# lh3/minigraph

Measured on NVIDIA H100. Metric: mapped Gbp/s (-cx lr), higher is better.
Workload: dtype int64/u8 (fp32 chain penalties, bit-exact)

## Files before the change

### minigraph_b200/csrc/mgb_common.cuh

```cuda
#pragma once
#include <stdint.h>
#include <stddef.h>
#include <string.h>

#if defined(__CUDACC__)
#define MG_HD __host__ __device__
#define MG_D __device__
#else
#define MG_HD
#define MG_D
#endif

#if defined(__CUDA_ARCH__)
#define MGB_ON_DEVICE 1
#else
#define MGB_ON_DEVICE 0
#endif

#if defined(__CUDACC__)
#define MG_NOINLINE __noinline__
#define MGB_NO_UNROLL _Pragma("unroll 1")
#else
#define MG_NOINLINE __attribute__((noinline))
#define MGB_NO_UNROLL
// ... 308 lines not shown
}
MG_HD inline int nth_set_bit(uint32_t mask, int k)
{
#if MGB_ON_DEVICE
	const unsigned r = __fns(mask, 0, k);
	return r > 31? 32 : (int)r;
#else
	for (int b = 0; b < 32; ++b) if ((mask >> b & 1) && --k == 0) return b;
	return 32;
#endif
}
MG_HD inline int replay_skips(uint32_t imp, uint32_t mk, int max_skip, int32_t *n_skip)
{
	int32_t ns = *n_skip;
	for (;;) {
		const int nxt = imp? ctz32_nz(imp) : 32;
		const uint32_t seg = nxt >= 32? mk : mk & ((1u << nxt) - 1u);
		const int c = mask_count(seg);
		if (ns + c > max_skip) { *n_skip = max_skip + 1; return nth_set_bit(seg, max_skip - ns + 1); }
		ns += c;
		if (nxt >= 32) break;
		if (ns > 0) --ns;
		imp &= imp - 1, mk &= ~((2u << nxt) - 1u);
	}
	*n_skip = ns;
	return -1;
}
MG_HD inline int ctz32(uint32_t x)
{
#if MGB_ON_DEVICE
	return __ffs((int)x) - 1;
#else
	return __builtin_ctz(x);
#endif
}

MG_HD inline int nt4(uint8_t c)
{
	const uint32_t idx = c & 0x1fu;
	const uint64_t code = (1ULL << 2 * 3) | (2ULL << 2 * 7) | (3ULL << 2 * 20) | (3ULL << 2 * 21);
	const uint32_t letters = (1u << 1) | (1u << 3) | (1u << 7) | (1u << 20) | (1u << 21);
	if ((c & 0xc0u) == 0x40u && (letters >> idx & 1u)) return (int)(code >> 2 * idx & 3u);
	return c < 4? (int)c : 4;
}

template<typename T, typename KeyFn>
MG_HD inline void rs_insertsort(T *beg, T *end, KeyFn key)
{
	for (T *i = beg + 1; i < end; ++i) {
		if (key(*i) < key(*(i - 1))) {
			T *j, tmp = *i;
			for (j = i; j > beg && key(tmp) < key(*(j - 1)); --j) *j = *(j - 1);
			*j = tmp;
		}
	}
}

struct RsRange { int32_t beg, end, s; };

template<typename T, typename KeyFn>
MG_HD inline int radix_sort_exact(Arena &A, T *a, int64_t n, int sizeof_key, KeyFn key)
{
	const int MIN_SIZE = 64;
	if (n <= MIN_SIZE) { rs_insertsort(a, a + n, key); return 0; }
	uint64_t mark = A.top;
	RsRange *stack;
// ... 205 lines not shown
```

### minigraph_b200/csrc/mgb_galign.cuh

```cuda
#pragma once
#include "mgb_pipeline.cuh"
#include "mgb_gchain.cuh"
#include "mgb_wfa_tiers.cuh"
#if defined(MGB_HOSTSIM)
#include <stdio.h>
#include <stdlib.h>
#endif

namespace mgb {

MG_HD inline int cigar_append1(Arena &A, AVec<uint64_t> &c, int32_t op, int32_t len)
{
	if (c.n > 0 && (int32_t)(c.a[c.n - 1] & 0xf) == op) c.a[c.n - 1] += (uint64_t)(int64_t)len << 4;
	else {
		uint64_t x = (uint64_t)(int64_t)len << 4 | (uint64_t)op;
		MGB_TRY(avec_push(A, c, x));
	}
	return 0;
}

MG_HD inline int cigar_append(Arena &A, AVec<uint64_t> &c, int32_t n_cigar, const uint32_t *cigar)
{
	if (n_cigar == 0) return 0;
	MGB_TRY(cigar_append1(A, c, (int32_t)(cigar[0] & 0xf), (int32_t)(cigar[0] >> 4)));
// ... 63 lines not shown
	const char *tseq;
	if (l == l0) tseq = g_vseq(g, lc[l0].v) + J->t_beg;
	else {
		char *seq;
		MGB_ALLOC(A, seq, char, tl + 1);
		int32_t n = g_vlen(g, lc[l0].v) - J->t_beg, at = 0;
		const char *s = g_vseq(g, lc[l0].v) + J->t_beg;
		for (int32_t x = lane; x < n; x += MGB_W) seq[at + x] = s[x];
		at += n;
		for (int32_t k = l0 + 1; k < l; ++k) {
			s = g_vseq(g, lc[k].v), n = g_vlen(g, lc[k].v);
			for (int32_t x = lane; x < n; x += MGB_W) seq[at + x] = s[x];
			at += n;
		}
		s = g_vseq(g, lc[l].v), n = J->t_last + 1;
		for (int32_t x = lane; x < n; x += MGB_W) seq[at + x] = s[x];
		at += n;
		if (at != tl) return MGB_E_INTERNAL;
		warp_sync();
		tseq = seq;
	}
	WfResult rst;
	unsigned long long pt0 = prof_clock();
	int rc;
	if (tier == 1) rc = wfa_smem<WfTier1::W_, WfTier1::MAXLEN_, WfTier1::TBCAP_>(A, smem, tl, tseq, ql, qs, &rst, lane);
	else if (tier == 2) rc = wfa_smem<WfTier2::W_, WfTier2::MAXLEN_, WfTier2::TBCAP_>(A, smem, tl, tseq, ql, qs, &rst, lane);
	else rc = wfa_exact(A, tl, tseq, ql, qs, 100000000LL, &rst, lane);
	if (rc < 0) return rc;
	if (lane == 0) {
		unsigned long long dt = prof_clock() - pt0;
		int slot = tier == 1? PROF_WFA_FAST_CYC : tier == 2? PROF_WFA_MID_CYC : PROF_WFA_SLOW_CYC;
		prof_add(c, slot, dt), prof_add(c, slot + 1, 1);
		prof_max(c, PROF_WFA_MAX_CYC, dt << 16 | (unsigned long long)(mlen < 65535? mlen : 65535));
		if (rc == 0) prof_add(c, PROF_WFA_CELLS, (unsigned long long)rst.n_iter);
		if (rc == 0 && explore && c.tier_hist) {
			unsigned int *h = &c.tier_hist[(mlen >> 4 < 31? mlen >> 4 : 31) * 4 + tier];
#if MGB_ON_DEVICE
			atomicAdd(h, 1u);
#else
			++*h;
#endif
		}
	}
	if (rc == 1) {
		if (lane == 0) {
			unsigned int at;
#if MGB_ON_DEVICE
			at = atomicAdd(&c.jobq_n[tier - 1], 1u);
#else
			at = c.jobq_n[tier - 1]++;
#endif
			c.jobq[tier - 1][at] = (int32_t)job_idx;
		}
		return 0;
	}
	if (rst.s < 0) return MGB_E_INTERNAL;
	int64_t coff = 0;
	if (lane == 0) {
#if MGB_ON_DEVICE
		unsigned long long *ck = wfa_cig_chunk(smem, tier);
		const unsigned long long need = ((unsigned long long)rst.n_cigar * 4 + 15) & ~15ULL;
		if (ck == 0) coff = pool_alloc(c.pool_cig, (uint64_t)rst.n_cigar * 4);
		else if (ck[0] + need > ck[1]) {
			const unsigned long long get = need > CIG_CHUNK_BYTES? need : CIG_CHUNK_BYTES;
			const int64_t off = pool_alloc(c.pool_cig, get);
			if (off < 0) ck[0] = ck[1] = 0;
			else ck[0] = (unsigned long long)off, ck[1] = (unsigned long long)off + get;
// ... 617 lines not shown
```

### minigraph_b200/csrc/mgb_pipeline.cuh

```cuda
#pragma once
#include "mgb_model.cuh"
#include "mgb_seed.cuh"
#include "mgb_lchain.cuh"
#include "mgb_gclabel.cuh"
#include "mgb_tma.cuh"

namespace mgb {

struct PipeCtx {
	GraphDev g;
	IndexDev ix;
	MapOptDev opt;
	BatchDev b;
	ReadMeta *meta;
	Pool *pool_anchor;     u128 *anchor;
	Pool *pool_minipos;    int32_t *minipos;
	Pool *pool_lchain;     LChain *lchain;
	Pool *pool_out;        char *out;
	Pool *pool_plan;       uint64_t *plan;
	Pool *pool_jobs;       struct WfaJob *jobs;
	Pool *pool_cig;        uint32_t *cig;
	int32_t *jobq[2];      unsigned int *jobq_n;
	Pool *pool_gstate;     char *gstate;
	Pool *pool_gjobs;      struct GwfaJob *gjobs;
	Pool *pool_walk;       int32_t *walk;
	int32_t *rescue_list;  unsigned int *rescue_n;
	LabTab lab;
	unsigned int *next_read;
	unsigned long long *prof;
	int32_t skip1_len, skip2_len;
	unsigned int *tier_hist;
};

enum { PROF_WFA_FAST_CYC = 0, PROF_WFA_FAST_N, PROF_WFA_SLOW_CYC, PROF_WFA_SLOW_N, PROF_WFA_MAX_CYC, PROF_WFA_CELLS, PROF_WFA_TB_CYC,
	   PROF_GC_DP_CYC, PROF_GC_GEN_CYC, PROF_GC_POST_CYC, PROF_GC_PLAN_CYC, PROF_FIN_CIGAR_CYC, PROF_FIN_DS_CYC, PROF_SEED_SKETCH_CYC,
	   PROF_SEED_MATCH_CYC, PROF_SEED_SORT_CYC, PROF_CHAIN_DP_CYC, PROF_CHAIN_BT_CYC, PROF_CHAIN_RMQ_CYC, PROF_CHAIN_POST_CYC, PROF_WFA_MID_CYC, PROF_WFA_MID_N, PROF_GC_GWFA_CYC, PROF_GC_SHORTK_CYC, PROF_GC_EXTRA_CYC, PROF_GWFA_MAX_CYC, PROF_GC_DP_MAX_CYC, PROF_WFA_CTA_CYC, PROF_WFA_CTA_N, PROF_LAB_CYC, PROF_LAB_N, PROF_N = 32 };

MG_HD inline unsigned long long prof_clock()
{
#if MGB_ON_DEVICE
	return (unsigned long long)clock64();
#else
	return 0;
#endif
}
#if defined(__CUDACC__)
MG_D inline unsigned long long *prof_block() { __shared__ unsigned long long s_prof[PROF_N]; return s_prof; }
MG_D inline bool prof_is_max(int slot) { return slot == PROF_WFA_MAX_CYC || slot == PROF_GWFA_MAX_CYC || slot == PROF_GC_DP_MAX_CYC; }
MG_D inline void prof_block_begin() { if (threadIdx.x < PROF_N) prof_block()[threadIdx.x] = 0; __syncthreads(); }
MG_D inline void prof_block_end(unsigned long long *prof)
{
	__syncthreads();
	if (prof && threadIdx.x < PROF_N) {
		const unsigned long long v = prof_block()[threadIdx.x];
		if (v) { if (prof_is_max((int)threadIdx.x)) atomicMax(&prof[threadIdx.x], v); else atomicAdd(&prof[threadIdx.x], v); }
	}
}
#endif
MG_HD inline void prof_add(const PipeCtx &c, int slot, unsigned long long v)
{
#if MGB_ON_DEVICE
	if (c.prof) atomicAdd(&prof_block()[slot], v);
#else
	if (c.prof) c.prof[slot] += v;
#endif
}
MG_HD inline void prof_max(const PipeCtx &c, int slot, unsigned long long v)
{
#if MGB_ON_DEVICE
	if (c.prof) atomicMax(&prof_block()[slot], v);
#else
	if (c.prof && c.prof[slot] < v) c.prof[slot] = v;
#endif
}

MG_HD inline int stage_seed(const PipeCtx &c, int rid, Arena &A, int lane, int32_t *smem = 0)
{
	ReadMeta &m = c.meta[rid];
// ... 281 lines not shown
```

### minigraph_b200/csrc/mgb_wfa.cuh

```cuda
#pragma once
#include "mgb_common.cuh"

namespace mgb {

static const int32_t WF_NEG_INF = -0x40000000;
static const int WF_X = 4, WF_O1 = 4, WF_E1 = 2, WF_O2 = 15, WF_E2 = 1;
static const int WF_MAX_PEN = 16;
static const int WF_NSLICE = WF_MAX_PEN + 1;
static const int WF_PAD = WF_MAX_PEN + 1;
static const int WF_SEQ_PAD = 16;

#define MGB_WF_MAX(a, b) ((a) >= (b)? (a) : (b))

struct WfResult {
	int32_t s;
	int32_t n_cigar;
	int64_t n_iter;
	uint32_t *cigar;
};


MG_HD inline void wf_stage_seq(char *dst, const char *src, int32_t len, uint8_t sentinel, int lane)
{
	for (int32_t i = lane; i < len; i += MGB_W) dst[i] = src[i];
	for (int32_t i = len + lane; i < len + WF_SEQ_PAD; i += MGB_W) dst[i] = (char)sentinel;
}

MG_HD inline uint32_t wf_ld32u(const char *base, int32_t pos)
{
	const uint32_t *w = (const uint32_t*)base;
	uint32_t lo = w[pos >> 2], hi = w[(pos >> 2) + 1];
	int sh = (pos & 3) << 3;
#if MGB_ON_DEVICE
	return __funnelshift_r(lo, hi, sh);
#else
	return sh? (lo >> sh) | (hi << (32 - sh)) : lo;
#endif
}

MG_HD inline int32_t wf_extend(const char *ts, const char *qs, int32_t k, int32_t d)
{
	for (;;) {
		uint32_t x = wf_ld32u(ts, k + 1) ^ wf_ld32u(qs, d + k + 1);
		if (x) {
#if MGB_ON_DEVICE
			return k + ((__ffs((int)x) - 1) >> 3);
#else
			return k + (__builtin_ctz(x) >> 3);
#endif
		}
		k += 4;
	}
}

template<typename TB>
MG_HD inline int wf_traceback(const TB &tb, int32_t n_scores, int32_t tl, const char *ts, int32_t ql, const char *qs, int32_t last_state,
							  uint32_t *cig_store, int64_t max_cigar, int32_t *n_cigar, int64_t *first)
{
	int32_t i = ql - 1, k = tl - 1, s = n_scores - 1, last = last_state;
	int64_t w = max_cigar;
	int32_t cur_op = -1, cur_len = 0;
#define MGB_CIG_PUSH(op_, len_) do { \
		if (cur_op == (op_)) cur_len += (len_); \
		else { \
			if (cur_op >= 0) { if (w <= 0) return MGB_E_INTERNAL; cig_store[--w] = (uint32_t)cur_len << 4 | (uint32_t)cur_op; } \
			cur_op = (op_), cur_len = (len_); \
		} \
	} while (0)
	while (i >= 0 && k >= 0) {
		int32_t k0 = k, x, state, ext;
		if (last == 0) {
			while (i >= 0 && k >= 0 && qs[i] == ts[k]) --i, --k;
			if (k0 - k > 0) MGB_CIG_PUSH(7, k0 - k);
			if (i < 0 || k < 0) break;
		}
		if (s < 0) return MGB_E_INTERNAL;
		x = tb.get(s, i - k);
		if (x < 0) return MGB_E_INTERNAL;
		state = last == 0? x & 7 : last;
		ext = state > 0? x >> (state + 2) & 1 : 0;
		if (state == 0) { MGB_CIG_PUSH(8, 1); --i, --k, s -= WF_X; }
		else if (state == 1) { MGB_CIG_PUSH(1, 1); --i, s -= ext? WF_E1 : WF_O1 + WF_E1; }
		else if (state == 3) { MGB_CIG_PUSH(1, 1); --i, s -= ext? WF_E2 : WF_O2 + WF_E2; }
		else if (state == 2) { MGB_CIG_PUSH(2, 1); --k, s -= ext? WF_E1 : WF_O1 + WF_E1; }
		else if (state == 4) { MGB_CIG_PUSH(2, 1); --k, s -= ext? WF_E2 : WF_O2 + WF_E2; }
		else return MGB_E_INTERNAL;
		last = state > 0 && ext? state : 0;
	}
	if (i >= 0) MGB_CIG_PUSH(1, i + 1);
	else if (k >= 0) MGB_CIG_PUSH(2, k + 1);
	if (cur_op >= 0) { if (w <= 0) return MGB_E_INTERNAL; cig_store[--w] = (uint32_t)cur_len << 4 | (uint32_t)cur_op; }
#undef MGB_CIG_PUSH
	*n_cigar = (int32_t)(max_cigar - w), *first = w;
	return 0;
}


typedef int16_t wf_cell_t;
static const int32_t WF_NEG_INF16 = -30000;

template<int W, int MAXLEN, int TBCAP, int HS = 17>
struct WfSmemLayout {
	static const int W_ = W, MAXLEN_ = MAXLEN, TBCAP_ = TBCAP, HS_ = HS;
	static const int N_CELLS = (HS + 3 + 3 + 2 + 2) * W;
	static const int N_INTS = N_CELLS / 2;
	static const int SEQ_BYTES = (MAXLEN + WF_SEQ_PAD + 3) / 4 * 4;
// ... 148 lines not shown
	x |= pHo2[d+1] >= pF2[d+1]? 0 : 0x40;
	f2 = MGB_WF_MAX(pHo2[d+1], pF2[d+1]) + 1;
	zf = f1 >= f2? 2 : 4;
	f = MGB_WF_MAX(f1, f2);
	z = e >= f? ze : zf;
	h = MGB_WF_MAX(e, f);
	z = pHx[d] + 1 >= h? 0 : z;
	E1[d] = e1, E2[d] = e2, F1[d] = f1, F2[d] = f2;
	H[d] = MGB_WF_MAX(pHx[d] + 1, h);
	return x | z;
}

struct WfChkpt { int32_t s, d; };

MG_HD inline int wfa_core(Arena &A, int32_t tl, const char *ts, int32_t ql, const char *qs, int64_t max_iter, int32_t n_seg, const WfChkpt *seg,
						  WfResult *r, uint32_t *cig_store, int64_t max_cigar, int lane, int nl)
{
	uint64_t mark = A.top;
	WfState wf;
	int32_t last_state = 0, stopped = 0, sid = 0;
	MGB_TRY(wf_state_alloc(A, wf, tl, ql));
	AVec<WfTbRow> rows;
	avec_init(rows);
	if (nl > 1) MGB_TRY(avec_reserve_w(A, rows, 1024, lane));
	else MGB_TRY(avec_reserve(A, rows, 1024));
	wf_stripe_init(wf, lane, nl);
	for (;;) {
		WfSlice *p = &wf.sl[wf.top];
		int32_t lo, hi, *H = p->H;
		int hit = 0, hit_noext = 0;
		for (int32_t d = p->lo + lane; d <= p->hi; d += nl) {
			int32_t k0 = H[d];
			if (k0 < -1 || d + k0 < -1 || k0 >= tl || d + k0 >= ql) continue;
			int32_t k = wf_extend(ts, qs, k0, d);
			if (k == tl - 1 && d + k == ql - 1) { hit = 1, hit_noext = (k == k0); if (nl == 1) break; }
			else H[d] = k;
		}
		MGB_NL_SYNC(nl);
		if (nl > 1? warp_any(hit) : hit) {
			if (nl > 1? warp_any(hit && hit_noext) : hit_noext) {
				WfTbArena t; t.row = rows.a;
				last_state = t.get((int32_t)rows.n - 1, ql - tl) & 7;
			}
			break;
		}
		if (seg && sid < n_seg && seg[sid].s == wf.s) {
			if (!(seg[sid].d >= wf.lo && seg[sid].d <= wf.hi)) { A.top = mark; return MGB_E_INTERNAL; }
			wf.lo = wf.hi = seg[sid++].d;
		}
		lo = wf.lo > -tl? wf.lo - 1 : -tl;
		hi = wf.hi < ql? wf.hi + 1 : ql;
		{
			const WfSlice &ft = wf_stripe_add(wf, lo, hi, lane, nl);
			const WfSlice &fx = wf_stripe_get(wf, WF_X);
			const WfSlice &fo1 = wf_stripe_get(wf, WF_O1 + WF_E1);
			const WfSlice &fo2 = wf_stripe_get(wf, WF_O2 + WF_E2);
			const WfSlice &fe1 = wf_stripe_get(wf, WF_E1);
			const WfSlice &fe2 = wf_stripe_get(wf, WF_E2);
			if (nl > 1) MGB_TRY(avec_reserve_w(A, rows, rows.n + 1, lane));
			else MGB_TRY(avec_reserve(A, rows, rows.n + 1));
			uint8_t *x;
			MGB_ALLOC(A, x, uint8_t, hi - lo + 1);
			if (lane == 0) rows.a[rows.n].lo = lo, rows.a[rows.n].hi = hi, rows.a[rows.n].x = x;
			++rows.n;
			uint8_t *ax = x - lo;
			for (int32_t dd = lo + lane; dd <= hi; dd += nl)
				ax[dd] = wf_cell(dd, ft.H, ft.E1, ft.F1, ft.E2, ft.F2, fx.H, fo1.H, fo2.H, fe1.E1, fe1.F1, fe2.E2, fe2.F2);
			MGB_NL_SYNC(nl);
			if (ft.H[lo] >= -1 || ft.E1[lo] >= -1 || ft.F1[lo] >= -1 || ft.E2[lo] >= -1 || ft.F2[lo] >= -1) wf.lo = lo;
			if (ft.H[hi] >= -1 || ft.E1[hi] >= -1 || ft.F1[hi] >= -1 || ft.E2[hi] >= -1 || ft.F2[hi] >= -1) wf.hi = hi;
		}
		if ((wf.s & 0xff) == 0) MGB_TRY(wf_stripe_shrink(wf, tl, ql));
		r->n_iter += hi - lo + 1;
		if (max_iter > 0 && r->n_iter > max_iter) { stopped = 1; break; }
	}
	r->s = stopped? -1 : wf.s;
	if (!stopped) {
		int rc = 0;
		int32_t n_cig = 0;
		int64_t first = 0;
		if (lane == 0) {
			WfTbArena t; t.row = rows.a;
			rc = wf_traceback(t, (int32_t)rows.n, tl, ts, ql, qs, last_state, cig_store, max_cigar, &n_cig, &first);
		}
		if (nl > 1) {
			rc = warp_bcast_i32(rc, 0), n_cig = warp_bcast_i32(n_cig, 0), first = (int64_t)warp_bcast_u64((uint64_t)first, 0);
			warp_sync();
		}
		if (rc < 0) { A.top = mark; return rc; }
		r->n_cigar = n_cig, r->cigar = cig_store + first;
	}
	A.top = mark;
	return 0;
}


struct WfSnap { int32_t n, n_intv, max_s; int32_t *x; uint64_t *intv; };

MG_HD inline int wf_snapshot(Arena &A, AVec<WfSnap> &sss, WfState &sf)
{
	WfSnap ss;
	int32_t j, k, t;
	ss.n = 0, ss.max_s = sf.s;
	for (j = 0; j < WF_NSLICE; ++j) ss.n += 5 * (sf.sl[j].hi - sf.sl[j].lo + 1);
	MGB_ALLOC(A, ss.x, int32_t, ss.n);
	ss.n_intv = WF_NSLICE;
	MGB_ALLOC(A, ss.intv, uint64_t, ss.n_intv);
	for (j = 0, t = 0; j < WF_NSLICE; ++j) {
		WfSlice *p = &sf.sl[(sf.top + 1 + j) % WF_NSLICE];
		ss.intv[j] = (uint64_t)(int64_t)p->lo << 32 | (uint64_t)(uint32_t)((p->hi - p->lo + 1) * 5);
		for (k = p->lo; k <= p->hi; ++k) {
			ss.x[t] = p->H[k],  p->H[k]  = t++;
			ss.x[t] = p->E1[k], p->E1[k] = t++;
			ss.x[t] = p->F1[k], p->F1[k] = t++;
			ss.x[t] = p->E2[k], p->E2[k] = t++;
			ss.x[t] = p->F2[k], p->F2[k] = t++;
		}
	}
	if (t != ss.n) return MGB_E_INTERNAL;
	return avec_push(A, sss, ss);
}

MG_HD inline int wfa_seg(Arena &A, int32_t step, int32_t tl, const char *ts, int32_t ql, const char *qs, WfChkpt **seg_, int32_t *n_seg_)
{
	uint64_t mark = A.top;
	WfState wf, sf;
	AVec<WfSnap> sss;
	uint8_t *xbuf;
	int32_t last = -1;
	avec_init(sss);
	*seg_ = 0, *n_seg_ = 0;
	MGB_ALLOC(A, xbuf, uint8_t, (int64_t)tl + ql + 1);
	MGB_TRY(wf_state_alloc(A, wf, tl, ql));
	MGB_TRY(wf_state_alloc(A, sf, tl, ql));
	wf_stripe_init(wf, 0, 1);
	wf_stripe_init(sf, 0, 1);
	for (;;) {
		WfSlice *p = &wf.sl[wf.top];
		int32_t d, lo, hi, *H = p->H;
		for (d = p->lo; d <= p->hi; ++d) {
			int32_t k0 = H[d];
			if (k0 < -1 || d + k0 < -1 || k0 >= tl || d + k0 >= ql) continue;
			int32_t k = wf_extend(ts, qs, k0, d);
			if (k == tl - 1 && d + k == ql - 1) { last = sf.sl[sf.top].H[d]; break; }
			H[d] = k;
		}
		if (d <= p->hi) break;
		lo = wf.lo > -tl? wf.lo - 1 : -tl;
		hi = wf.hi < ql? wf.hi + 1 : ql;
		if ((wf.s + 1) % step == 0) MGB_TRY(wf_snapshot(A, sss, sf));
		{
			uint8_t *ax = xbuf - lo;
			{
				const WfSlice &ft = wf_stripe_add(wf, lo, hi, 0, 1);
				const WfSlice &fx = wf_stripe_get(wf, WF_X), &fo1 = wf_stripe_get(wf, WF_O1 + WF_E1), &fo2 = wf_stripe_get(wf, WF_O2 + WF_E2);
				const WfSlice &fe1 = wf_stripe_get(wf, WF_E1), &fe2 = wf_stripe_get(wf, WF_E2);
				for (int32_t dd = lo; dd <= hi; ++dd)
					ax[dd] = wf_cell(dd, ft.H, ft.E1, ft.F1, ft.E2, ft.F2, fx.H, fo1.H, fo2.H, fe1.E1, fe1.F1, fe2.E2, fe2.F2);
			}
			const WfSlice &gt = wf_stripe_add(sf, lo, hi, 0, 1);
			const WfSlice &gx = wf_stripe_get(sf, WF_X), &go1 = wf_stripe_get(sf, WF_O1 + WF_E1), &go2 = wf_stripe_get(sf, WF_O2 + WF_E2);
			const WfSlice &ge1 = wf_stripe_get(sf, WF_E1), &ge2 = wf_stripe_get(sf, WF_E2);
			for (int32_t dd = lo; dd <= hi; ++dd) {
				uint8_t x = ax[dd];
				int32_t e1, f1, e2, f2, h;
				e1 = gt.E1[dd] = (x & 0x08) == 0? go1.H[dd-1] : ge1.E1[dd-1];
				f1 = gt.F1[dd] = (x & 0x10) == 0? go1.H[dd+1] : ge1.F1[dd+1];
				e2 = gt.E2[dd] = (x & 0x20) == 0? go2.H[dd-1] : ge2.E2[dd-1];
				f2 = gt.F2[dd] = (x & 0x40) == 0? go2.H[dd+1] : ge2.F2[dd+1];
				x &= 7;
				h = gx.H[dd];
				h = x == 1? e1 : h;
				h = x == 2? f1 : h;
				h = x == 3? e2 : h;
				h = x == 4? f2 : h;
				gt.H[dd] = h;
// ... 221 lines not shown
				}
				r->s += q.s;
				A.top = m2;
			}
		} else if (x0 < x1) {
			MGB_TRY(wf_cig_push1(cig_store, &nc, max_cigar, 2, x1 - x0));
			r->s += WF_O2 + (x1 - x0) * WF_E2 < WF_O1 + (x1 - x0) * WF_E1? WF_O2 + (x1 - x0) * WF_E2 : WF_O1 + (x1 - x0) * WF_E1;
		} else if (y0 < y1) {
			MGB_TRY(wf_cig_push1(cig_store, &nc, max_cigar, 1, y1 - y0));
			r->s += WF_O2 + (y1 - y0) * WF_E2 < WF_O1 + (y1 - y0) * WF_E1? WF_O2 + (y1 - y0) * WF_E2 : WF_O1 + (y1 - y0) * WF_E1;
		}
		x0 = x1, y0 = y1;
	}
	A.top = mark;
	r->n_cigar = (int32_t)nc, r->cigar = cig_store;
	return 0;
}


MG_HD inline int wfa_ring_g(Arena &A, int32_t tl, const char *ts, int32_t ql, const char *qs, int64_t max_iter, WfResult *r,
							 uint32_t *cig_store, int64_t max_cigar, int lane);
MG_HD MG_NOINLINE inline int wfa_core_cold(Arena &A, int32_t tl, const char *ts, int32_t ql, const char *qs, int64_t max_iter, WfResult *r, uint32_t *cig_store, int64_t max_cigar, int lane)
{
	return wfa_core(A, tl, ts, ql, qs, max_iter, 0, 0, r, cig_store, max_cigar, lane, MGB_W);
}
MG_HD MG_NOINLINE inline int wfa_chain_cold(Arena &A, int32_t tl, const char *ts_g, int32_t ql, const char *qs_g, WfResult *r, uint32_t *cig_store, int64_t max_cigar, int32_t step)
{
	return wfa_chain(A, tl, ts_g, ql, qs_g, r, cig_store, max_cigar, step);
}

MG_HD inline int wfa_exact(Arena &A, int32_t tl, const char *ts_g, int32_t ql, const char *qs_g, int64_t max_iter, WfResult *r, int lane, int32_t step = 5000)
{
	uint64_t mark = A.top;
	r->s = -1, r->n_cigar = 0, r->n_iter = 0, r->cigar = 0;
	uint32_t *cig_store;
	const int64_t max_cigar = (int64_t)tl + ql + 2;
	MGB_ALLOC(A, cig_store, uint32_t, max_cigar);
	uint64_t mark_keep = A.top;
	char *ts, *qs;
	MGB_ALLOC(A, ts, char, tl + WF_SEQ_PAD + 4);
	MGB_ALLOC(A, qs, char, ql + WF_SEQ_PAD + 4);
	wf_stage_seq(ts, ts_g, tl, 0xfe, lane);
	wf_stage_seq(qs, qs_g, ql, 0xff, lane);
	warp_sync();
	{
		int rc = wfa_ring_g(A, tl, ts, ql, qs, max_iter, r, cig_store, max_cigar, lane);
		if (rc < 0) return rc;
		if (rc == 1) {
			Arena B = A;
			rc = wfa_core_cold(B, tl, ts, ql, qs, max_iter, r, cig_store, max_cigar, lane);
			A.top = B.top, A.peak = B.peak;
			if (rc < 0) return rc;
		}
	}
	if (r->s < 0) {
		int rc = 0;
		int32_t n_cig = 0, sc = 0;
		if (lane == 0) {
			Arena B = A;
			rc = wfa_chain_cold(B, tl, ts_g, ql, qs_g, r, cig_store, max_cigar, step);
			n_cig = r->n_cigar, sc = r->s;
			if (B.peak > A.peak) A.peak = B.peak;
		}
		rc = warp_bcast_i32(rc, 0), n_cig = warp_bcast_i32(n_cig, 0), sc = warp_bcast_i32(sc, 0);
		warp_sync();
		if (rc < 0) { A.top = mark; return rc; }
		r->s = sc, r->n_cigar = n_cig, r->cigar = cig_store;
// ... 10 lines not shown
```

### minigraph_b200/csrc/mgb_wfa_tiers.cuh

```cuda
#pragma once
#include "mgb_wfa.cuh"

namespace mgb {

#if MGB_ON_DEVICE
MG_D inline uint32_t warp_or_u32(uint32_t x) { return __reduce_or_sync(0xffffffffu, x); }
#elif defined(MGB_SIM_LANES)
inline uint32_t warp_or_u32(uint32_t x) { uint64_t o[32]; sim::exchange(x, o, 15); uint32_t r = 0; for (int i = 0; i < MGB_W; ++i) r |= (uint32_t)o[i]; return r; }
#else
inline uint32_t warp_or_u32(uint32_t x) { return x; }
#endif

#define MGB_OPAQUE(x) asm("" : "+r"(x))

MG_HD inline int32_t wf2_ld(const void *base, int32_t off)
{
	int32_t v = *(const wf_cell_t*)((const char*)base + off);
	MGB_OPAQUE(v);
	return v;
}

#define MGB_WF_CELL_LOAD(S, d_) \
	int32_t h##S, e1##S, e2##S, f1##S, f2##S; \
	uint8_t xz##S; \
	const int32_t c##S = (((d_) + (1 << 20)) * 2) & colmask2;  \
	{ \
		const int32_t cm_ = (c##S - 2) & colmask2, cp_ = (c##S + 2) & colmask2; \
		int32_t a0_, b0_, e_, f_; \
		uint8_t x_ = 0, ze_, zf_, z_; \
		a0_ = wf2_ld(H, bHo1 + cm_), b0_ = wf2_ld(E1, bE1 + cm_); \
		x_ |= a0_ >= b0_? 0 : 0x08; e1##S = MGB_WF_MAX(a0_, b0_); \
		a0_ = wf2_ld(H, bHo2 + cm_), b0_ = wf2_ld(E2, bE2 + cm_); \
		x_ |= a0_ >= b0_? 0 : 0x20; e2##S = MGB_WF_MAX(a0_, b0_); \
		ze_ = e1##S >= e2##S? 1 : 3; \
		e_ = MGB_WF_MAX(e1##S, e2##S); \
		a0_ = wf2_ld(H, bHo1 + cp_), b0_ = wf2_ld(F1, bE1 + cp_); \
		x_ |= a0_ >= b0_? 0 : 0x10; f1##S = MGB_WF_MAX(a0_, b0_) + 1; \
		a0_ = wf2_ld(H, bHo2 + cp_), b0_ = wf2_ld(F2, bE2 + cp_); \
		x_ |= a0_ >= b0_? 0 : 0x40; f2##S = MGB_WF_MAX(a0_, b0_) + 1; \
		zf_ = f1##S >= f2##S? 2 : 4; \
		f_ = MGB_WF_MAX(f1##S, f2##S); \
		z_ = e_ >= f_? ze_ : zf_; \
		h##S = MGB_WF_MAX(e_, f_); \
		a0_ = wf2_ld(H, bHx + c##S) + 1; \
		z_ = a0_ >= h##S? 0 : z_; \
		h##S = MGB_WF_MAX(a0_, h##S); \
		xz##S = x_ | z_; \
	}
#define MGB_WF_CELL_FINISH(S, d_) \
	{ \
		const int32_t dd_ = (d_); \
		ax[dd_] = xz##S; \
		if (dd_ == lo || dd_ == hi) {  \
			if (h##S >= -1 || e1##S >= -1 || f1##S >= -1 || e2##S >= -1 || f2##S >= -1) vote |= (dd_ == lo? 1u : 0u) | (dd_ == hi? 2u : 0u); \
		} \
		if (!(h##S < -1 || dd_ + h##S < -1 || h##S >= tl || dd_ + h##S >= ql)) {  \
			const int32_t k_ = wf_extend(ts, qs, h##S, dd_); \
			if (dd_ == d_corner && k_ == tl - 1) vote |= 4u | (k_ == h##S? 8u : 0u); \
			else h##S = k_; \
		} \
		*(wf_cell_t*)((char*)E1 + bn3 + c##S) = (wf_cell_t)e1##S, *(wf_cell_t*)((char*)F1 + bn3 + c##S) = (wf_cell_t)f1##S; \
		*(wf_cell_t*)((char*)E2 + bn2 + c##S) = (wf_cell_t)e2##S, *(wf_cell_t*)((char*)F2 + bn2 + c##S) = (wf_cell_t)f2##S; \
		*(wf_cell_t*)((char*)H + bnH + c##S) = (wf_cell_t)h##S; \
	}

template<int W, int MAXLEN, int TBCAP>
MG_HD inline int wfa_smem(Arena &A, int32_t *smem, int32_t tl, const char *ts_g, int32_t ql, const char *qs_g, WfResult *r, int lane)
{
	typedef WfSmemLayout<W, MAXLEN, TBCAP, 17> LY;
	const int HS = 17;
	if (tl > MAXLEN || ql > MAXLEN) return 1;
	if (MAXLEN > 16000) return 1;
	uint64_t mark = A.top;
	wf_cell_t *H = (wf_cell_t*)smem, *E1 = H + HS * W, *F1 = E1 + 3 * W, *E2 = F1 + 3 * W, *F2 = E2 + 2 * W;
	char *ts = (char*)(smem + LY::N_INTS), *qs = ts + LY::SEQ_BYTES;
	int32_t *tb_row = (int32_t*)(qs + LY::SEQ_BYTES);
	uint8_t *tb_x = (uint8_t*)tb_row + LY::TB_ROW_BYTES;
	{
		const uint32_t two = (uint32_t)(uint16_t)(wf_cell_t)WF_NEG_INF16 * 0x10001u;
		uint32_t *cells = (uint32_t*)smem;
		for (int32_t i = lane; i < LY::N_INTS; i += MGB_W) cells[i] = two;
	}
	wf_stage_seq(ts, ts_g, tl, 0xfe, lane);
	wf_stage_seq(qs, qs_g, ql, 0xff, lane);
	r->s = -1, r->n_cigar = 0, r->n_iter = 0, r->cigar = 0;
	uint32_t *cig_store;
	const int64_t max_cigar = (int64_t)tl + ql + 2;
	MGB_ALLOC(A, cig_store, uint32_t, max_cigar);
	uint64_t mark_keep = A.top;
	AVec<WfTbRow> rows;
	avec_init(rows);
	if (TBCAP == 0) MGB_TRY(avec_reserve_w(A, rows, 256, lane));
	int32_t n_rows = 0, tb_used = 0;
	int32_t wlo = 0, whi = 0, last_state = 0, s = 0;
	int64_t n_iter = 0;
	int hs = 0, m3 = 0, m2 = 0;
	const int32_t d_corner = ql - tl;
	int hit = 0, hit_noext = 0;
	warp_sync();
	if (lane == 0) {
		int32_t k0 = -1, k = -1;
		if (!(k0 >= tl || k0 >= ql)) {
			k = wf_extend(ts, qs, k0, 0);
			if (k == tl - 1 && k == ql - 1) hit = 1, hit_noext = (k == k0), k = k0;
		}
		H[wfs_col<W>(0)] = (wf_cell_t)k;
	}
	{
		const uint32_t vb = warp_or_u32((hit? 1u : 0u) | (hit_noext? 2u : 0u));
		hit = vb & 1, hit_noext = vb >> 1 & 1;
	}
	warp_sync();
	for (;;) {
		if (hit) {
			if (hit_noext) {
				int32_t x;
				if (TBCAP > 0) { WfTbSmem t; t.row = tb_row, t.x = tb_x, t.n_rows = n_rows, t.used = tb_used; x = t.get(n_rows - 1, ql - tl); }
				else { WfTbArena t; t.row = rows.a; x = t.get(n_rows - 1, ql - tl); }
				last_state = x & 7;
			}
			break;
		}
		const int32_t lo = wlo > -tl? wlo - 1 : -tl;
		const int32_t hi = whi < ql? whi + 1 : ql;
		const int32_t width = hi - lo + 1;
		if (width + 2 > W || s + 1 >= 255 || (TBCAP > 0 && tb_used + width > TBCAP)) { A.top = mark; return 1; }
		const int32_t ns = s + 1;
		const int nhs = hs + 1 == 17? 0 : hs + 1, n3 = m3 + 1 == 3? 0 : m3 + 1, n2 = m2 ^ 1;
		uint8_t *ax;
		if (TBCAP > 0) {
			if (lane == 0) tb_row[2 * n_rows] = lo, tb_row[2 * n_rows + 1] = tb_used;
			ax = tb_x + tb_used - lo;
			tb_used += width;
		} else {
			uint8_t *x;
			MGB_ALLOC(A, x, uint8_t, width);
			if (lane == 0) rows.a[n_rows].lo = lo, rows.a[n_rows].hi = hi, rows.a[n_rows].x = x;
			rows.n = n_rows + 1;
			ax = x - lo;
		}
		++n_rows;
		const int r4 = nhs >= WF_X? nhs - WF_X : nhs - WF_X + 17, r6 = nhs >= WF_O1 + WF_E1? nhs - (WF_O1 + WF_E1) : nhs - (WF_O1 + WF_E1) + 17;
		const int r16 = nhs >= WF_O2 + WF_E2? nhs - (WF_O2 + WF_E2) : nhs - (WF_O2 + WF_E2) + 17;
		const int e1slot = n3 >= 2? n3 - 2 : n3 + 1;
		int32_t bHx = r4 * W * 2, bHo1 = r6 * W * 2, bHo2 = r16 * W * 2, bE1 = e1slot * W * 2, bE2 = m2 * W * 2, bnH = nhs * W * 2, bn3 = n3 * W * 2, bn2 = n2 * W * 2;
		MGB_OPAQUE(bHx); MGB_OPAQUE(bHo1); MGB_OPAQUE(bHo2); MGB_OPAQUE(bE1); MGB_OPAQUE(bE2); MGB_OPAQUE(bnH); MGB_OPAQUE(bn3); MGB_OPAQUE(bn2);
		const int32_t colmask2 = 2 * W - 1;
		uint32_t vote = 0;
		for (int32_t d = lo + lane; d <= hi; d += MGB_W) {
			MGB_WF_CELL_LOAD(A, d)
			MGB_WF_CELL_FINISH(A, d)
		}
		vote = warp_or_u32(vote);
		if (vote & 1) wlo = lo;
		if (vote & 2) whi = hi;
		hit = vote >> 2 & 1, hit_noext = vote >> 3 & 1;
		s = ns, hs = nhs, m3 = n3, m2 = n2;
		n_iter += width;
		warp_sync();
	}
	r->n_iter = n_iter;
	r->s = s;
	{
		int rc = 0;
		int32_t n_cig = 0;
		int64_t first = 0;
		if (lane == 0) {
			if (TBCAP > 0) { WfTbSmem t; t.row = tb_row, t.x = tb_x, t.n_rows = n_rows, t.used = tb_used; rc = wf_traceback(t, n_rows, tl, ts, ql, qs, last_state, cig_store, max_cigar, &n_cig, &first); }
			else { WfTbArena t; t.row = rows.a; rc = wf_traceback(t, n_rows, tl, ts, ql, qs, last_state, cig_store, max_cigar, &n_cig, &first); }
		}
		rc = warp_bcast_i32(rc, 0), n_cig = warp_bcast_i32(n_cig, 0), first = (int64_t)warp_bcast_u64((uint64_t)first, 0);
		warp_sync();
		if (rc < 0) { A.top = mark; return rc; }
		r->n_cigar = n_cig, r->cigar = cig_store + first;
	}
	A.top = mark_keep;
	return 0;
}

static const int WF3_NSL = 17 + 3 + 3 + 2 + 2 + 1;
#define MGB_WF2_FILL(need_lo_, need_hi_) do { \
		const int32_t nl_ = (need_lo_), nh_ = (need_hi_); \
		if (fhi < flo || nl_ < flo || nh_ > fhi) { \
			int32_t tlo_ = nl_ - 128 > -tl - 1? nl_ - 128 : -tl - 1, thi_ = nh_ + 128 < ql + 1? nh_ + 128 : ql + 1; \
			if (fhi >= flo) { if (nl_ >= flo) tlo_ = flo; if (nh_ <= fhi) thi_ = fhi; } \
			const int32_t a0_ = tlo_, a1_ = fhi >= flo? flo - 1 : thi_, b0_ = fhi >= flo? fhi + 1 : thi_ + 1, b1_ = thi_; \
			for (int sl_ = 0; sl_ < WF3_NSL; ++sl_) { \
				wf_cell_t *p_ = cells + (int64_t)sl_ * W; \
				for (int32_t d_ = a0_ + lane; d_ <= a1_; d_ += MGB_W) p_[(d_ + (1 << 20)) & mask] = (wf_cell_t)WF_NEG_INF16; \
				for (int32_t d_ = b0_ + lane; d_ <= b1_; d_ += MGB_W) p_[(d_ + (1 << 20)) & mask] = (wf_cell_t)WF_NEG_INF16; \
			} \
			flo = tlo_, fhi = thi_; \
			warp_sync(); \
		} \
	} while (0)
#define MGB_WF2_CLEAN(p_, g_) do { \
		const int32_t olo_ = (int32_t)((g_) & 0xffffu) - 0x8000, ohi_ = (int32_t)((g_) >> 16) - 0x8000; \
		if (olo_ < lo || ohi_ > hi) { \
			wf_cell_t *q_ = (p_); \
			for (int32_t d_ = olo_ + lane; d_ <= ohi_ && d_ < lo; d_ += MGB_W) q_[(d_ + (1 << 20)) & mask] = (wf_cell_t)WF_NEG_INF16; \
			for (int32_t d_ = (hi + 1 > olo_? hi + 1 : olo_) + lane; d_ <= ohi_; d_ += MGB_W) q_[(d_ + (1 << 20)) & mask] = (wf_cell_t)WF_NEG_INF16; \
		} \
// ... 5 lines not shown
	if (tl + ql > 16000 || tl <= 0 || ql <= 0) return 1;
	uint64_t mark = A.top;
	int32_t W = 64;
	while (W < tl + ql + 2) W <<= 1;
	const int32_t mask = W - 1;
	wf_cell_t *cells;
	MGB_ALLOC(A, cells, wf_cell_t, (int64_t)WF3_NSL * W);
	wf_cell_t *H = cells, *E1 = H + 17 * W, *F1 = E1 + 3 * W, *E2 = F1 + 3 * W, *F2 = E2 + 2 * W, *G = F2 + 2 * W;
	int32_t flo = 0, fhi = -1;
	const int32_t d_corner = ql - tl;
	AVec<WfTbRow> rows;
	avec_init(rows);
	MGB_TRY(avec_reserve_w(A, rows, 1024, lane));
	int32_t n_rows = 0;
	int32_t wlo = 0, whi = 0, last_state = 0, s = 0, stopped = 0;
	int64_t n_iter = 0;
	int hs = 0, m3 = 0, m2 = 0;
#define MGB_WF_RG(lo_, hi_) ((uint32_t)((hi_) + 0x8000) << 16 | (uint32_t)((lo_) + 0x8000))
#if MGB_W >= 32
	uint32_t g_mine = lane == 0? MGB_WF_RG(0, 0) : MGB_WF_RG(1, 0);
#define MGB_WF_GGET(slot_) ((uint32_t)warp_bcast_i32((int32_t)g_mine, (slot_)))
#define MGB_WF_GSET(slot_, v_) do { if (lane == (slot_)) g_mine = (v_); } while (0)
#else
	uint32_t g_all[17];
	for (int j = 0; j < 17; ++j) g_all[j] = j == 0? MGB_WF_RG(0, 0) : MGB_WF_RG(1, 0);
#define MGB_WF_GGET(slot_) (g_all[(slot_)])
#define MGB_WF_GSET(slot_, v_) (g_all[(slot_)] = (v_))
#endif
	int hit = 0, hit_noext = 0;
	MGB_WF2_FILL(-1, 1);
	if (lane == 0) {
		const int32_t c0 = (1 << 20) & mask;
		int32_t k0 = -1, k = -1;
		k = wf_extend(ts, qs, k0, 0);
		if (k == tl - 1 && k == ql - 1) hit = 1, hit_noext = (k == k0), k = k0;
		H[c0] = (wf_cell_t)k;
	}
	{
		const uint32_t vb = warp_or_u32((hit? 1u : 0u) | (hit_noext? 2u : 0u));
		hit = vb & 1, hit_noext = vb >> 1 & 1;
	}
	warp_sync();
	for (;;) {
		if (hit) {
			if (hit_noext) { WfTbArena t; t.row = rows.a; last_state = t.get(n_rows - 1, ql - tl) & 7; }
			break;
		}
		const int32_t lo = wlo > -tl? wlo - 1 : -tl;
		const int32_t hi = whi < ql? whi + 1 : ql;
		const int32_t width = hi - lo + 1;
		const int32_t ns = s + 1;
		const int nhs = hs + 1 == 17? 0 : hs + 1, n3 = m3 + 1 == 3? 0 : m3 + 1, n2 = m2 ^ 1;
		MGB_TRY(avec_reserve_w(A, rows, n_rows + 1, lane));
		uint8_t *x;
		MGB_ALLOC(A, x, uint8_t, width);
		if (lane == 0) rows.a[n_rows].lo = lo, rows.a[n_rows].hi = hi, rows.a[n_rows].x = x;
		rows.n = ++n_rows;
		uint8_t *ax = x - lo;
		const int r4 = nhs >= WF_X? nhs - WF_X : nhs - WF_X + 17, r6 = nhs >= WF_O1 + WF_E1? nhs - (WF_O1 + WF_E1) : nhs - (WF_O1 + WF_E1) + 17;
		const int r16 = nhs >= WF_O2 + WF_E2? nhs - (WF_O2 + WF_E2) : nhs - (WF_O2 + WF_E2) + 17;
		const int e1slot = n3 >= 2? n3 - 2 : n3 + 1;
		MGB_WF2_FILL(lo - 1, hi + 1);
		const uint32_t g16 = MGB_WF_GGET(nhs), g2 = MGB_WF_GGET(nhs >= 3? nhs - 3 : nhs + 14), g1 = MGB_WF_GGET(nhs >= 2? nhs - 2 : nhs + 15);
		MGB_WF2_CLEAN(H + (int64_t)nhs * W, g16);
		MGB_WF2_CLEAN(E1 + (int64_t)n3 * W, g2);
		MGB_WF2_CLEAN(F1 + (int64_t)n3 * W, g2);
		MGB_WF2_CLEAN(E2 + (int64_t)n2 * W, g1);
		MGB_WF2_CLEAN(F2 + (int64_t)n2 * W, g1);
		int32_t bHx = r4 * W * 2, bHo1 = r6 * W * 2, bHo2 = r16 * W * 2, bE1 = e1slot * W * 2, bE2 = m2 * W * 2, bnH = nhs * W * 2, bn3 = n3 * W * 2, bn2 = n2 * W * 2;
		MGB_OPAQUE(bHx); MGB_OPAQUE(bHo1); MGB_OPAQUE(bHo2); MGB_OPAQUE(bE1); MGB_OPAQUE(bE2); MGB_OPAQUE(bnH); MGB_OPAQUE(bn3); MGB_OPAQUE(bn2);
		const int track = ((ns + 16) & 0xff) <= 16;
		uint32_t vote = 0;
		const int32_t colmask2 = 2 * W - 1;
#define MGB_WF_TRACK(S, d_) do { if (track && (wf_good_diag((d_), h##S, tl, ql) || wf_good_diag((d_), e1##S, tl, ql) || wf_good_diag((d_), f1##S, tl, ql) || wf_good_diag((d_), e2##S, tl, ql) || wf_good_diag((d_), f2##S, tl, ql))) \
				*(wf_cell_t*)((char*)G + c##S) = (wf_cell_t)ns; } while (0)
		for (int32_t d = lo + lane; d <= hi; d += 2 * MGB_W) {
			const int32_t dB = d + MGB_W <= hi? d + MGB_W : d;
			MGB_WF_CELL_LOAD(A, d)
			MGB_WF_CELL_LOAD(B, dB)
			MGB_WF_CELL_FINISH(A, d)
			MGB_WF_TRACK(A, d);
			if (dB != d) { MGB_WF_CELL_FINISH(B, dB) MGB_WF_TRACK(B, dB); }
		}
#undef MGB_WF_TRACK
		vote = warp_or_u32(vote);
		if (vote & 1) wlo = lo;
		if (vote & 2) whi = hi;
		hit = vote >> 2 & 1, hit_noext = vote >> 3 & 1;
		MGB_WF_GSET(nhs, MGB_WF_RG(lo, hi));
		s = ns, hs = nhs, m3 = n3, m2 = n2;
		warp_sync();
		if ((s & 0xff) == 0) {
			int32_t nlo = 0, nhi = 0, found = 0;
			for (int pass = 0; pass < 2; ++pass) {
				found = 0;
				for (int32_t base = pass == 0? wlo : whi; pass == 0? base <= whi : base >= wlo; base += pass == 0? MGB_W : -MGB_W) {
					const int32_t d = pass == 0? base + lane : base - lane;
					int good = 0;
					if (d >= wlo && d <= whi) good = G[(d + (1 << 20)) & mask] >= s - 16;
					const uint32_t m = warp_ballot(good);
					if (m) { found = 1; if (pass == 0) nlo = base + ctz32(m); else nhi = base - ctz32(m); break; }
				}
				if (!found) break;
			}
			if (!found) { A.top = mark; return MGB_E_INTERNAL; }
			wlo = nlo, whi = nhi;
		}
		n_iter += width;
		if (max_iter > 0 && n_iter > max_iter) { stopped = 1; break; }
	}
#undef MGB_WF_RG
#undef MGB_WF_GGET
#undef MGB_WF_GSET
	r->n_iter = n_iter;
	r->s = stopped? -1 : s;
	if (!stopped) {
		int rc = 0;
		int32_t n_cig = 0;
		int64_t first = 0;
		if (lane == 0) {
			WfTbArena t; t.row = rows.a;
			rc = wf_traceback(t, n_rows, tl, ts, ql, qs, last_state, cig_store, max_cigar, &n_cig, &first);
		}
		rc = warp_bcast_i32(rc, 0), n_cig = warp_bcast_i32(n_cig, 0), first = (int64_t)warp_bcast_u64((uint64_t)first, 0);
		warp_sync();
		if (rc < 0) { A.top = mark; return rc; }
		r->n_cigar = n_cig, r->cigar = cig_store + first;
	}
	A.top = mark;
	return 0;
}
#undef MGB_WF2_CLEAN
#undef MGB_WF2_FILL


}
```

Measured before the change: 1.330.

## Pack WFA shared-memory sequences to 2-bit codes for wider match extension

The shared-memory WFA tier stages the target and query into a 2-bit packed form when both contain only ACGT, and falls back to byte staging otherwise. Diagonal extension and the traceback match scan then compare 16 bases per 32-bit word instead of 4, with explicit end-of-sequence limits in place of sentinel bytes. The traceback match run now scans whole words backwards using clz. The change also adds traceback cycle profiling. It costs a per-character validation and a warp vote during staging, and it adds bounds arithmetic to each extension call.

```diff
diff --git a/minigraph_b200/csrc/mgb_common.cuh b/minigraph_b200/csrc/mgb_common.cuh
--- a/minigraph_b200/csrc/mgb_common.cuh
+++ b/minigraph_b200/csrc/mgb_common.cuh
@@ -364,6 +364,24 @@
 	return __ffs((int)x) - 1;
 #else
 	return __builtin_ctz(x);
+#endif
+}
+
+MG_HD inline int clz32(uint32_t x)
+{
+#if MGB_ON_DEVICE
+	return __clz((int)x);
+#else
+	return __builtin_clz(x);
+#endif
+}
+
+MG_HD inline unsigned long long prof_clock()
+{
+#if MGB_ON_DEVICE
+	return (unsigned long long)clock64();
+#else
+	return 0;
 #endif
 }
 
diff --git a/minigraph_b200/csrc/mgb_galign.cuh b/minigraph_b200/csrc/mgb_galign.cuh
--- a/minigraph_b200/csrc/mgb_galign.cuh
+++ b/minigraph_b200/csrc/mgb_galign.cuh
@@ -119,7 +119,7 @@
 		int slot = tier == 1? PROF_WFA_FAST_CYC : tier == 2? PROF_WFA_MID_CYC : PROF_WFA_SLOW_CYC;
 		prof_add(c, slot, dt), prof_add(c, slot + 1, 1);
 		prof_max(c, PROF_WFA_MAX_CYC, dt << 16 | (unsigned long long)(mlen < 65535? mlen : 65535));
-		if (rc == 0) prof_add(c, PROF_WFA_CELLS, (unsigned long long)rst.n_iter);
+		if (rc == 0) prof_add(c, PROF_WFA_CELLS, (unsigned long long)rst.n_iter), prof_add(c, PROF_WFA_TB_CYC, rst.tb_cyc);
 		if (rc == 0 && explore && c.tier_hist) {
 			unsigned int *h = &c.tier_hist[(mlen >> 4 < 31? mlen >> 4 : 31) * 4 + tier];
 #if MGB_ON_DEVICE
diff --git a/minigraph_b200/csrc/mgb_pipeline.cuh b/minigraph_b200/csrc/mgb_pipeline.cuh
--- a/minigraph_b200/csrc/mgb_pipeline.cuh
+++ b/minigraph_b200/csrc/mgb_pipeline.cuh
@@ -36,14 +36,6 @@
 	   PROF_GC_DP_CYC, PROF_GC_GEN_CYC, PROF_GC_POST_CYC, PROF_GC_PLAN_CYC, PROF_FIN_CIGAR_CYC, PROF_FIN_DS_CYC, PROF_SEED_SKETCH_CYC,
 	   PROF_SEED_MATCH_CYC, PROF_SEED_SORT_CYC, PROF_CHAIN_DP_CYC, PROF_CHAIN_BT_CYC, PROF_CHAIN_RMQ_CYC, PROF_CHAIN_POST_CYC, PROF_WFA_MID_CYC, PROF_WFA_MID_N, PROF_GC_GWFA_CYC, PROF_GC_SHORTK_CYC, PROF_GC_EXTRA_CYC, PROF_GWFA_MAX_CYC, PROF_GC_DP_MAX_CYC, PROF_WFA_CTA_CYC, PROF_WFA_CTA_N, PROF_LAB_CYC, PROF_LAB_N, PROF_N = 32 };
 
-MG_HD inline unsigned long long prof_clock()
-{
-#if MGB_ON_DEVICE
-	return (unsigned long long)clock64();
-#else
-	return 0;
-#endif
-}
 #if defined(__CUDACC__)
 MG_D inline unsigned long long *prof_block() { __shared__ unsigned long long s_prof[PROF_N]; return s_prof; }
 MG_D inline bool prof_is_max(int slot) { return slot == PROF_WFA_MAX_CYC || slot == PROF_GWFA_MAX_CYC || slot == PROF_GC_DP_MAX_CYC; }
diff --git a/minigraph_b200/csrc/mgb_wfa.cuh b/minigraph_b200/csrc/mgb_wfa.cuh
--- a/minigraph_b200/csrc/mgb_wfa.cuh
+++ b/minigraph_b200/csrc/mgb_wfa.cuh
@@ -17,6 +17,7 @@
 	int32_t n_cigar;
 	int64_t n_iter;
 	uint32_t *cigar;
+	unsigned long long tb_cyc;
 };
 
 
@@ -26,11 +27,43 @@
 	for (int32_t i = len + lane; i < len + WF_SEQ_PAD; i += MGB_W) dst[i] = (char)sentinel;
 }
 
-MG_HD inline uint32_t wf_ld32u(const char *base, int32_t pos)
+MG_HD inline int wf_stage_2b(char *dst, const char *src, int32_t len, int lane)
+{
+	uint32_t *w = (uint32_t*)dst;
+	int ok = 1;
+	for (int32_t j = lane; j < ((len + 15) >> 4) + 2; j += MGB_W) {
+		const int32_t n = len - 16 * j;
+		uint32_t x = 0;
+#if defined(__CUDACC__)
+#pragma unroll
+#endif
+		for (int t = 0; t < 16; ++t) {
+			if (t < n) {
+				const uint32_t c = (uint8_t)src[16 * j + t], b = (c >> 1 ^ c >> 2) & 3u;
+				ok &= (0x54474341u >> 8 * b & 0xffu) == c;
+				x |= b << 2 * t;
+			}
+		}
+		w[j] = x;
+	}
+	return ok;
+}
+
+MG_HD inline int wf_stage_pair(char *ts, const char *ts_g, int32_t tl, char *qs, const char *qs_g, int32_t ql, int lane)
+{
+	const int ok = wf_stage_2b(ts, ts_g, tl, lane) & wf_stage_2b(qs, qs_g, ql, lane);
+	if (!warp_any(!ok)) return 1;
+	warp_sync();
+	wf_stage_seq(ts, ts_g, tl, 0xfe, lane);
+	wf_stage_seq(qs, qs_g, ql, 0xff, lane);
+	return 3;
+}
+
+MG_HD inline uint32_t wf_ld_bits(const char *base, int32_t bit)
 {
 	const uint32_t *w = (const uint32_t*)base;
-	uint32_t lo = w[pos >> 2], hi = w[(pos >> 2) + 1];
-	int sh = (pos & 3) << 3;
+	uint32_t lo = w[bit >> 5], hi = w[(bit >> 5) + 1];
+	int sh = bit & 31;
 #if MGB_ON_DEVICE
 	return __funnelshift_r(lo, hi, sh);
 #else
@@ -38,23 +71,32 @@
 #endif
 }
 
-MG_HD inline int32_t wf_extend(const char *ts, const char *qs, int32_t k, int32_t d)
+MG_HD inline uint32_t wf_ld_bits_below(const char *base, int32_t end)
+{
+	return end >= 32? wf_ld_bits(base, end - 32) : ((const uint32_t*)base)[0] << (32 - end);
+}
+
+MG_HD inline int32_t wf_extend(const char *ts, const char *qs, int32_t k, int32_t d, int32_t lim, int lb)
 {
 	for (;;) {
-		uint32_t x = wf_ld32u(ts, k + 1) ^ wf_ld32u(qs, d + k + 1);
-		if (x) {
-#if MGB_ON_DEVICE
-			return k + ((__ffs((int)x) - 1) >> 3);
-#else
-			return k + (__builtin_ctz(x) >> 3);
-#endif
-		}
+		const uint32_t x = wf_ld_bits(ts, (k + 1) << lb) ^ wf_ld_bits(qs, (d + k + 1) << lb);
+		if (x) { k += ctz32(x) >> lb; return k < lim? k : lim; }
+		k += 32 >> lb;
+		if (k >= lim) return lim;
+	}
+}
+
+MG_HD inline int32_t wf_extend_bytes(const char *ts, const char *qs, int32_t k, int32_t d)
+{
+	for (;;) {
+		const uint32_t x = wf_ld_bits(ts, (k + 1) << 3) ^ wf_ld_bits(qs, (d + k + 1) << 3);
+		if (x) return k + (ctz32(x) >> 3);
 		k += 4;
 	}
 }
 
 template<typename TB>
-MG_HD inline int wf_traceback(const TB &tb, int32_t n_scores, int32_t tl, const char *ts, int32_t ql, const char *qs, int32_t last_state,
+MG_HD inline int wf_traceback(const TB &tb, int32_t n_scores, int32_t tl, const char *ts, int32_t ql, const char *qs, int lb, int32_t last_state,
 							  uint32_t *cig_store, int64_t max_cigar, int32_t *n_cigar, int64_t *first)
 {
 	int32_t i = ql - 1, k = tl - 1, s = n_scores - 1, last = last_state;
@@ -68,10 +110,19 @@
 		} \
 	} while (0)
 	while (i >= 0 && k >= 0) {
-		int32_t k0 = k, x, state, ext;
+		int32_t x, state, ext;
 		if (last == 0) {
-			while (i >= 0 && k >= 0 && qs[i] == ts[k]) --i, --k;
-			if (k0 - k > 0) MGB_CIG_PUSH(7, k0 - k);
+			const int32_t n = (i < k? i : k) + 1;
+			int32_t m = 0;
+			for (;;) {
+				const uint32_t y = wf_ld_bits_below(qs, (i - m + 1) << lb) ^ wf_ld_bits_below(ts, (k - m + 1) << lb);
+				if (y) { m += clz32(y) >> lb; break; }
+				m += 32 >> lb;
+				if (m >= n) break;
+			}
+			if (m > n) m = n;
+			i -= m, k -= m;
+			if (m > 0) MGB_CIG_PUSH(7, m);
 			if (i < 0 || k < 0) break;
 		}
 		if (s < 0) return MGB_E_INTERNAL;
@@ -286,7 +337,7 @@
 		for (int32_t d = p->lo + lane; d <= p->hi; d += nl) {
 			int32_t k0 = H[d];
 			if (k0 < -1 || d + k0 < -1 || k0 >= tl || d + k0 >= ql) continue;
-			int32_t k = wf_extend(ts, qs, k0, d);
+			int32_t k = wf_extend_bytes(ts, qs, k0, d);
 			if (k == tl - 1 && d + k == ql - 1) { hit = 1, hit_noext = (k == k0); if (nl == 1) break; }
 			else H[d] = k;
 		}
@@ -335,7 +386,7 @@
 		int64_t first = 0;
 		if (lane == 0) {
 			WfTbArena t; t.row = rows.a;
-			rc = wf_traceback(t, (int32_t)rows.n, tl, ts, ql, qs, last_state, cig_store, max_cigar, &n_cig, &first);
+			rc = wf_traceback(t, (int32_t)rows.n, tl, ts, ql, qs, 3, last_state, cig_store, max_cigar, &n_cig, &first);
 		}
 		if (nl > 1) {
 			rc = warp_bcast_i32(rc, 0), n_cig = warp_bcast_i32(n_cig, 0), first = (int64_t)warp_bcast_u64((uint64_t)first, 0);
@@ -395,7 +446,7 @@
 		for (d = p->lo; d <= p->hi; ++d) {
 			int32_t k0 = H[d];
 			if (k0 < -1 || d + k0 < -1 || k0 >= tl || d + k0 >= ql) continue;
-			int32_t k = wf_extend(ts, qs, k0, d);
+			int32_t k = wf_extend_bytes(ts, qs, k0, d);
 			if (k == tl - 1 && d + k == ql - 1) { last = sf.sl[sf.top].H[d]; break; }
 			H[d] = k;
 		}
@@ -683,7 +734,7 @@
 MG_HD inline int wfa_exact(Arena &A, int32_t tl, const char *ts_g, int32_t ql, const char *qs_g, int64_t max_iter, WfResult *r, int lane, int32_t step = 5000)
 {
 	uint64_t mark = A.top;
-	r->s = -1, r->n_cigar = 0, r->n_iter = 0, r->cigar = 0;
+	r->s = -1, r->n_cigar = 0, r->n_iter = 0, r->cigar = 0, r->tb_cyc = 0;
 	uint32_t *cig_store;
 	const int64_t max_cigar = (int64_t)tl + ql + 2;
 	MGB_ALLOC(A, cig_store, uint32_t, max_cigar);
diff --git a/minigraph_b200/csrc/mgb_wfa_tiers.cuh b/minigraph_b200/csrc/mgb_wfa_tiers.cuh
--- a/minigraph_b200/csrc/mgb_wfa_tiers.cuh
+++ b/minigraph_b200/csrc/mgb_wfa_tiers.cuh
@@ -55,7 +55,7 @@
 			if (h##S >= -1 || e1##S >= -1 || f1##S >= -1 || e2##S >= -1 || f2##S >= -1) vote |= (dd_ == lo? 1u : 0u) | (dd_ == hi? 2u : 0u); \
 		} \
 		if (!(h##S < -1 || dd_ + h##S < -1 || h##S >= tl || dd_ + h##S >= ql)) {  \
-			const int32_t k_ = wf_extend(ts, qs, h##S, dd_); \
+			const int32_t k_ = MGB_WF_EXTEND(h##S, dd_); \
 			if (dd_ == d_corner && k_ == tl - 1) vote |= 4u | (k_ == h##S? 8u : 0u); \
 			else h##S = k_; \
 		} \
@@ -81,9 +81,8 @@
 		uint32_t *cells = (uint32_t*)smem;
 		for (int32_t i = lane; i < LY::N_INTS; i += MGB_W) cells[i] = two;
 	}
-	wf_stage_seq(ts, ts_g, tl, 0xfe, lane);
-	wf_stage_seq(qs, qs_g, ql, 0xff, lane);
-	r->s = -1, r->n_cigar = 0, r->n_iter = 0, r->cigar = 0;
+	const int lb = wf_stage_pair(ts, ts_g, tl, qs, qs_g, ql, lane);
+	r->s = -1, r->n_cigar = 0, r->n_iter = 0, r->cigar = 0, r->tb_cyc = 0;
 	uint32_t *cig_store;
 	const int64_t max_cigar = (int64_t)tl + ql + 2;
 	MGB_ALLOC(A, cig_store, uint32_t, max_cigar);
@@ -101,7 +100,7 @@
 	if (lane == 0) {
 		int32_t k0 = -1, k = -1;
 		if (!(k0 >= tl || k0 >= ql)) {
-			k = wf_extend(ts, qs, k0, 0);
+			k = wf_extend(ts, qs, k0, 0, (tl < ql? tl : ql) - 1, lb);
 			if (k == tl - 1 && k == ql - 1) hit = 1, hit_noext = (k == k0), k = k0;
 		}
 		H[wfs_col<W>(0)] = (wf_cell_t)k;
@@ -147,10 +146,12 @@
 		MGB_OPAQUE(bHx); MGB_OPAQUE(bHo1); MGB_OPAQUE(bHo2); MGB_OPAQUE(bE1); MGB_OPAQUE(bE2); MGB_OPAQUE(bnH); MGB_OPAQUE(bn3); MGB_OPAQUE(bn2);
 		const int32_t colmask2 = 2 * W - 1;
 		uint32_t vote = 0;
+#define MGB_WF_EXTEND(k_, d_) wf_extend(ts, qs, (k_), (d_), tl - 1 < ql - 1 - (d_)? tl - 1 : ql - 1 - (d_), lb)
 		for (int32_t d = lo + lane; d <= hi; d += MGB_W) {
 			MGB_WF_CELL_LOAD(A, d)
 			MGB_WF_CELL_FINISH(A, d)
 		}
+#undef MGB_WF_EXTEND
 		vote = warp_or_u32(vote);
 		if (vote & 1) wlo = lo;
 		if (vote & 2) whi = hi;
@@ -166,8 +167,10 @@
 		int32_t n_cig = 0;
 		int64_t first = 0;
 		if (lane == 0) {
-			if (TBCAP > 0) { WfTbSmem t; t.row = tb_row, t.x = tb_x, t.n_rows = n_rows, t.used = tb_used; rc = wf_traceback(t, n_rows, tl, ts, ql, qs, last_state, cig_store, max_cigar, &n_cig, &first); }
-			else { WfTbArena t; t.row = rows.a; rc = wf_traceback(t, n_rows, tl, ts, ql, qs, last_state, cig_store, max_cigar, &n_cig, &first); }
+			const unsigned long long t0 = prof_clock();
+			if (TBCAP > 0) { WfTbSmem t; t.row = tb_row, t.x = tb_x, t.n_rows = n_rows, t.used = tb_used; rc = wf_traceback(t, n_rows, tl, ts, ql, qs, lb, last_state, cig_store, max_cigar, &n_cig, &first); }
+			else { WfTbArena t; t.row = rows.a; rc = wf_traceback(t, n_rows, tl, ts, ql, qs, lb, last_state, cig_store, max_cigar, &n_cig, &first); }
+			r->tb_cyc = prof_clock() - t0;
 		}
 		rc = warp_bcast_i32(rc, 0), n_cig = warp_bcast_i32(n_cig, 0), first = (int64_t)warp_bcast_u64((uint64_t)first, 0);
 		warp_sync();
@@ -239,7 +242,7 @@
 	if (lane == 0) {
 		const int32_t c0 = (1 << 20) & mask;
 		int32_t k0 = -1, k = -1;
-		k = wf_extend(ts, qs, k0, 0);
+		k = wf_extend_bytes(ts, qs, k0, 0);
 		if (k == tl - 1 && k == ql - 1) hit = 1, hit_noext = (k == k0), k = k0;
 		H[c0] = (wf_cell_t)k;
 	}
@@ -281,6 +284,7 @@
 		const int32_t colmask2 = 2 * W - 1;
 #define MGB_WF_TRACK(S, d_) do { if (track && (wf_good_diag((d_), h##S, tl, ql) || wf_good_diag((d_), e1##S, tl, ql) || wf_good_diag((d_), f1##S, tl, ql) || wf_good_diag((d_), e2##S, tl, ql) || wf_good_diag((d_), f2##S, tl, ql))) \
 				*(wf_cell_t*)((char*)G + c##S) = (wf_cell_t)ns; } while (0)
+#define MGB_WF_EXTEND(k_, d_) wf_extend_bytes(ts, qs, (k_), (d_))
 		for (int32_t d = lo + lane; d <= hi; d += 2 * MGB_W) {
 			const int32_t dB = d + MGB_W <= hi? d + MGB_W : d;
 			MGB_WF_CELL_LOAD(A, d)
@@ -289,6 +293,7 @@
 			MGB_WF_TRACK(A, d);
 			if (dB != d) { MGB_WF_CELL_FINISH(B, dB) MGB_WF_TRACK(B, dB); }
 		}
+#undef MGB_WF_EXTEND
 #undef MGB_WF_TRACK
 		vote = warp_or_u32(vote);
 		if (vote & 1) wlo = lo;
@@ -326,8 +331,10 @@
 		int32_t n_cig = 0;
 		int64_t first = 0;
 		if (lane == 0) {
+			const unsigned long long t0 = prof_clock();
 			WfTbArena t; t.row = rows.a;
-			rc = wf_traceback(t, n_rows, tl, ts, ql, qs, last_state, cig_store, max_cigar, &n_cig, &first);
+			rc = wf_traceback(t, n_rows, tl, ts, ql, qs, 3, last_state, cig_store, max_cigar, &n_cig, &first);
+			r->tb_cyc = prof_clock() - t0;
 		}
 		rc = warp_bcast_i32(rc, 0), n_cig = warp_bcast_i32(n_cig, 0), first = (int64_t)warp_bcast_u64((uint64_t)first, 0);
 		warp_sync();
```

New measurement: 1.337 (median of 6 runs). Within noise of the previous version (+0.6%).
